# idiap/IdiapTTS

Hardware: AMD Instinct MI355X
Metric: acoustic frames/sec (train) (higher is better)
Workload: dtype f32

## Files before the change

idiaptts_amd/csrc/nn.hip:

```cpp
#include <algorithm>
#include <cstdlib>

#include "common.h"
#include "gemm_ring.h"
#include "gemm_staged.h"

namespace itts {

constexpr int BN = 128;

template <bool ROWFORM, bool VEC, int NROWS>
__device__ __forceinline__ void load_tile(const float* __restrict__ P, int64_t ld, int64_t out0,
                                          int64_t out_dim, int64_t k0, int64_t k_end,
                                          float4 (&r)[NROWS / 32]) {
  const int tid = threadIdx.x;
#pragma unroll
  for (int i = 0; i < NROWS / 32; ++i) {
    const int idx = tid + 256 * i;
    int64_t o, k;
    if (ROWFORM) {
      o = out0 + (idx >> 3);
      k = k0 + ((idx & 7) << 2);
    } else {
      k = k0 + idx / (NROWS / 4);
      o = out0 + ((idx % (NROWS / 4)) << 2);
    }
    const int64_t c = ROWFORM ? k : o, c_end = ROWFORM ? k_end : out_dim;
    const int64_t t = ROWFORM ? o : k, t_end = ROWFORM ? out_dim : k_end;
    const bool t_ok = t < t_end;
    const int64_t tc = t_ok ? t : 0;
    if (VEC) {
      const bool ok = t_ok && (c < c_end);
      const float4 v = *reinterpret_cast<const float4*>(P + tc * ld + (ok ? c : 0));
// ... 219 lines not shown
static int ring_wm(int64_t M, int N) {
  const double w2 = (double)(((M + 127) / 128) * 128) * (double)(((N + 63) / 64) * 64);
  const double w1 = (double)(((M + 63) / 64) * 64) * (double)(((N + 127) / 128) * 128);
  return w1 < w2 ? 1 : 2;
}

template <bool A_ROW, bool B_ROW, int EPI, int AF>
static int launch_ring(const GemmArgs& g, int splitk, hipStream_t s) {
  if (ring_wm(g.M, g.N) == 1) return launch_ring_wm<A_ROW, B_ROW, EPI, 1, AF>(g, splitk, s);
  return launch_ring_wm<A_ROW, B_ROW, EPI, 2, AF>(g, splitk, s);
}

template <int WM_W, int EPI_X, int AF_X = AF_BASE>
static int launch_ring_bwd_pair(const GemmArgs& gw, int splitk, const GemmArgs& gx, hipStream_t s) {
  const ring::Args rw = ring_args<WM_W>(gw, splitk), rx = ring_args<2>(gx, 1);
  hipLaunchKernelGGL((ring::gemm_ring_pair_kernel<false, false, EPI_STORE, WM_W, true, false, EPI_X, 2, AF_X>),
                     dim3(kRingGrid), dim3(ring::THREADS), 0, s, rw, rx);
  ITTS_LAUNCH_CHECK();
  return ITTS_OK;
}

template <bool A_ROW, bool B_ROW, int EPI, int AF = AF_BASE>
static int launch_gemm(GemmArgs g, int splitk, hipStream_t s) {
  if (g.M <= 0 || g.N <= 0) return ITTS_OK;
  if (ring_ok<A_ROW, B_ROW>(g, splitk, EPI)) return launch_ring<A_ROW, B_ROW, EPI, AF>(g, splitk, s);
  if (A_ROW) return launch_gemm_tn<A_ROW, B_ROW, EPI, 1, 1, AF>(g, splitk, s);
  const double e2 = tile_efficiency(g.M, g.N, splitk, 2, 1.0);
  const double e1 = tile_efficiency(g.M, g.N, splitk, 1, 0.90);
  if (e1 > e2) return launch_gemm_tn<A_ROW, B_ROW, EPI, 1, 2, AF>(g, splitk, s);
  return launch_gemm_tn<A_ROW, B_ROW, EPI, 2, 2, AF>(g, splitk, s);
}


__device__ __forceinline__ void reduce_slabs_vec_body(const float* __restrict__ slabs, int S, int64_t n,
                                                      float* __restrict__ out, int accumulate, int64_t block,
                                                      float4 (*part)[64]) {
  const int tx = threadIdx.x & 63, grp = threadIdx.x >> 6;
  const int64_t n4 = n >> 2;
  const int64_t c = block * 64 + tx;
  float4 s = make_float4(0.f, 0.f, 0.f, 0.f);
  if (c < n4) {
    const float4* p = reinterpret_cast<const float4*>(slabs) + c;
#pragma unroll 8
    for (int z = grp; z < S; z += 4) {
      const float4 v = p[(int64_t)z * n4];
      s.x += v.x; s.y += v.y; s.z += v.z; s.w += v.w;
    }
  }
  if (grp > 0) part[grp - 1][tx] = s;
  __syncthreads();
  if (grp == 0 && c < n4) {
#pragma unroll
    for (int g2 = 0; g2 < 3; ++g2) {
      const float4 v = part[g2][tx];
      s.x += v.x; s.y += v.y; s.z += v.z; s.w += v.w;
    }
    float4* o = reinterpret_cast<float4*>(out) + c;
    if (accumulate) {
      const float4 v = *o;
      s.x += v.x; s.y += v.y; s.z += v.z; s.w += v.w;
    }
    *o = s;
  }
}

__device__ __forceinline__ void reduce_slabs_scalar_body(const float* __restrict__ slabs, int S, int64_t n,
                                                         float* __restrict__ out, int accumulate,
                                                         int64_t block, float (*part)[64]) {
  const int tx = threadIdx.x & 63, grp = threadIdx.x >> 6;
  const int64_t c = block * 64 + tx;
  float s = 0.f;
  if (c < n) {
#pragma unroll 8
    for (int z = grp; z < S; z += 4) s += slabs[(int64_t)z * n + c];
  }
  if (grp > 0) part[grp - 1][tx] = s;
  __syncthreads();
  if (grp == 0 && c < n) {
    s += part[0][tx];
    s += part[1][tx];
    s += part[2][tx];
    out[c] = accumulate ? out[c] + s : s;
  }
}

__global__ __launch_bounds__(256) void reduce_slabs_kernel(const float* __restrict__ slabs, int S,
                                                           int64_t n, float* __restrict__ out,
                                                           int accumulate) {
  __shared__ float4 part[3][64];
  reduce_slabs_vec_body(slabs, S, n, out, accumulate, blockIdx.x, part);
}

__global__ __launch_bounds__(256) void reduce_slabs_scalar_kernel(const float* __restrict__ slabs, int S,
                                                                  int64_t n, float* __restrict__ out,
                                                                  int accumulate) {
  __shared__ float part[3][64];
  reduce_slabs_scalar_body(slabs, S, n, out, accumulate, blockIdx.x, part);
}

constexpr int kMaxDeferred = 16;
struct ReduceSeg {
  const void* src;
  void* out;
  int64_t n;
  double scale;
  int S;
  int accumulate;
  int kind;
  int first_block;
};
struct ReduceMulti {
  ReduceSeg seg[kMaxDeferred];
  int nseg;
};

__global__ __launch_bounds__(256) void reduce_multi_kernel(ReduceMulti d) {
  __shared__ float4 part4[3][64];
  __shared__ double red[16];
  int i = 0;
  while (i + 1 < d.nseg && (int)blockIdx.x >= d.seg[i + 1].first_block) ++i;
  const ReduceSeg& g = d.seg[i];
  const int64_t block = (int64_t)blockIdx.x - g.first_block;
  if (g.kind == 0) {
    reduce_slabs_vec_body(static_cast<const float*>(g.src), g.S, g.n, static_cast<float*>(g.out), g.accumulate,
                          block, part4);
  } else if (g.kind == 1) {
    reduce_slabs_scalar_body(static_cast<const float*>(g.src), g.S, g.n, static_cast<float*>(g.out),
                             g.accumulate, block, reinterpret_cast<float (*)[64]>(part4));
  } else {
    const double* partial = static_cast<const double*>(g.src);
    double s = 0.0;
    for (int k = threadIdx.x; k < (int)g.n; k += 256) s += partial[k];
    s = block_sum(s, red);
    if (threadIdx.x == 0) *static_cast<float*>(g.out) = (float)(s * g.scale);
  }
}

static thread_local bool t_defer = false;
static thread_local ReduceMulti t_pending{};

static int flush_deferred(hipStream_t s) {
  if (t_pending.nseg == 0) return ITTS_OK;
  const ReduceSeg& last = t_pending.seg[t_pending.nseg - 1];
  const int64_t per = last.kind == 0 ? (last.n / 4 + 63) / 64 : (last.kind == 1 ? (last.n + 63) / 64 : 1);
  const int64_t blocks = last.first_block + per;
  hipLaunchKernelGGL(reduce_multi_kernel, dim3((unsigned)blocks), dim3(256), 0, s, t_pending);
  t_pending.nseg = 0;
  ITTS_LAUNCH_CHECK();
  return ITTS_OK;
}

static int queue_deferred(ReduceSeg g, hipStream_t s) {
  if (t_pending.nseg == kMaxDeferred) {
    const int rc = flush_deferred(s);
    if (rc) return rc;
  }
  int64_t first = 0;
  if (t_pending.nseg > 0) {
    const ReduceSeg& p = t_pending.seg[t_pending.nseg - 1];
    first = p.first_block + (p.kind == 0 ? (p.n / 4 + 63) / 64 : (p.kind == 1 ? (p.n + 63) / 64 : 1));
  }
  ITTS_REQUIRE(first < ((int64_t)1 << 30), "too many deferred reduction blocks");
  g.first_block = (int)first;
  t_pending.seg[t_pending.nseg++] = g;
  return ITTS_OK;
}

static int launch_reduce_slabs(const float* slabs, int S, int64_t n, float* out, int accumulate,
                               hipStream_t s) {
  const bool vec = n % 4 == 0 && aligned16(slabs) && aligned16(out);
  if (t_defer) {
    ReduceSeg g{};
    g.src = slabs; g.out = out; g.n = n; g.S = S; g.accumulate = accumulate; g.kind = vec ? 0 : 1;
    return queue_deferred(g, s);
  }
  if (vec)
    hipLaunchKernelGGL(reduce_slabs_kernel, dim3((unsigned)((n / 4 + 63) / 64)), dim3(256), 0, s, slabs, S,
                       n, out, accumulate);
  else
    hipLaunchKernelGGL(reduce_slabs_scalar_kernel, dim3((unsigned)((n + 63) / 64)), dim3(256), 0, s, slabs,
                       S, n, out, accumulate);
  ITTS_LAUNCH_CHECK();
  return ITTS_OK;
}

extern "C" int itts_defer_reductions(int on) {
  ITTS_REQUIRE(on || t_pending.nseg == 0,
               "queued reductions must be run (itts_reduce_deferred) before deferral is switched off");
  t_defer = on != 0;
  return ITTS_OK;
}

extern "C" int itts_reduce_deferred(void* stream) {
  t_defer = false;
  return flush_deferred(as_stream(stream));
}

template <int AF>
__global__ void act_bwd_kernel(const float* __restrict__ dy, const float* __restrict__ y,
                               float* __restrict__ dz, int64_t n, int act) {
  if (AF == AF_BASE) {
    for (int64_t i = blockIdx.x * (int64_t)blockDim.x + threadIdx.x; i < n;
         i += (int64_t)gridDim.x * blockDim.x)
      dz[i] = dy[i] * act_grad_from_out(y[i], act);
  } else {
    with_ext_act(act, [&](auto a) {
      for (int64_t i = blockIdx.x * (int64_t)blockDim.x + threadIdx.x; i < n;
           i += (int64_t)gridDim.x * blockDim.x)
        dz[i] = dy[i] * dact1<decltype(a)::value>(y[i]);
    });
  }
}

__global__ __launch_bounds__(256) void masked_mse_kernel(
    const float* __restrict__ pred, int64_t ldp, const float* __restrict__ target, int64_t ldt,
    const uint8_t* __restrict__ valid, int64_t M, int D, float gscale, float* __restrict__ grad,
    int64_t ldg, double* __restrict__ partial) {
  __shared__ double red[16];
  const int64_t n = M * D;
  double s = 0.0;
  for (int64_t i = blockIdx.x * (int64_t)blockDim.x + threadIdx.x; i < n;
       i += (int64_t)gridDim.x * blockDim.x) {
    const int64_t r = i / D;
    const int c = (int)(i - r * D);
    float diff = 0.f;
    if (valid[r]) diff = pred[r * ldp + c] - target[r * ldt + c];
    s += (double)diff * (double)diff;
    if (grad) grad[r * ldg + c] = gscale * diff;
// ... 16 lines not shown
  if (t_defer) {
    ReduceSeg g{};
    g.src = partial; g.out = loss; g.n = nb; g.scale = scale; g.S = 1; g.kind = 2;
    return queue_deferred(g, s);
  }
  hipLaunchKernelGGL(masked_mse_final_kernel, dim3(1), dim3(256), 0, s, partial, nb, scale, loss);
  ITTS_LAUNCH_CHECK();
  return ITTS_OK;
}


__global__ __launch_bounds__(256) void weighted_loss_kernel(
    const float* __restrict__ pred, int64_t ldp, const float* __restrict__ target, int64_t ldt,
    const float* __restrict__ w, int64_t M, int D, int kind, float* __restrict__ grad, int64_t ldg,
    float* __restrict__ elem, int64_t lde, double* __restrict__ partial) {
  __shared__ double red[16];
  const int64_t n = M * D;
  double s = 0.0;
  for (int64_t i = blockIdx.x * (int64_t)blockDim.x + threadIdx.x; i < n;
       i += (int64_t)gridDim.x * blockDim.x) {
    const int64_t r = i / D;
    const int c = (int)(i - r * D);
    const float wr = w[r];
    const float diff = pred[r * ldp + c] - target[r * ldt + c];
    const float e = kind == 0 ? diff * diff : fabsf(diff);
    const float g = kind == 0 ? 2.f * diff : (diff > 0.f ? 1.f : (diff < 0.f ? -1.f : 0.f));
    const float v = wr == 0.f ? 0.f : wr * e;
    s += (double)v;
    if (grad) grad[r * ldg + c] = wr == 0.f ? 0.f : wr * g;
    if (elem) elem[r * lde + c] = v;
  }
  s = block_sum(s, red);
  if (threadIdx.x == 0) partial[blockIdx.x] = s;
}

__global__ void adam_kernel(float* __restrict__ p, const float* __restrict__ g,
                            float* __restrict__ m, float* __restrict__ v, int64_t n, float beta1,
                            float beta2, float eps, float wd, float step_size, float bc2_sqrt,
                            float gscale) {
  for (int64_t i = blockIdx.x * (int64_t)blockDim.x + threadIdx.x; i < n;
       i += (int64_t)gridDim.x * blockDim.x) {
    float gi = g[i] * gscale;
    float pi = p[i];
    if (wd != 0.f) gi += wd * pi;
    float mi = m[i], vi = v[i];
    mi = mi + (gi - mi) * (1.f - beta1);
    vi = vi * beta2 + (1.f - beta2) * gi * gi;
    const float denom = sqrtf(vi) / bc2_sqrt + eps;
    pi = pi - step_size * (mi / denom);
    p[i] = pi;
    m[i] = mi;
    v[i] = vi;
  }
}

__global__ void adam_fused_kernel(float* __restrict__ p, const float* __restrict__ g,
                                  float* __restrict__ m, float* __restrict__ v, int64_t n,
                                  float beta1, float beta2, float eps, float wd, float step_size,
                                  float bc2_sqrt, float gscale, const float* __restrict__ norm_accum,
                                  int norm_kind, float max_norm, float clip_value,
                                  float* __restrict__ shadow, float one_minus_decay) {
  float coef = gscale;
  if (norm_accum) {
    const float a = norm_accum[0];
    const float total = (norm_kind == 2 ? sqrtf(a) : a) * fabsf(gscale);
    coef *= fminf(1.f, max_norm / (total + 1e-6f));
  }
  for (int64_t i = blockIdx.x * (int64_t)blockDim.x + threadIdx.x; i < n;
       i += (int64_t)gridDim.x * blockDim.x) {
    float gi = g[i] * coef;
    if (clip_value > 0.f) gi = fminf(fmaxf(gi, -clip_value), clip_value);
    float pi = p[i];
    if (wd != 0.f) gi += wd * pi;
    float mi = m[i], vi = v[i];
    mi = mi + (gi - mi) * (1.f - beta1);
    vi = vi * beta2 + (1.f - beta2) * gi * gi;
    const float denom = sqrtf(vi) / bc2_sqrt + eps;
    pi = pi - step_size * (mi / denom);
    p[i] = pi;
    m[i] = mi;
    v[i] = vi;
    if (shadow) {
      const float si = shadow[i];
      shadow[i] = si - one_minus_decay * (si - pi);
    }
  }
// ... 360 lines not shown
  return launch_mse_final(reinterpret_cast<const double*>(d_workspace), nb, scale, d_loss, s);
}

extern "C" int itts_weighted_loss(const float* d_pred, int64_t ldp, const float* d_target, int64_t ldt,
                                  const float* d_row_weight, int64_t M, int D, int kind,
                                  float* d_loss, float* d_grad, int64_t ldg, float* d_elem,
                                  int64_t lde, void* d_workspace, void* stream) {
  ITTS_REQUIRE(d_pred && d_target && d_row_weight && d_loss && d_workspace, "null pointer");
  ITTS_REQUIRE(M >= 0 && D > 0 && ldp >= D && ldt >= D && (kind == 0 || kind == 1), "bad sizes");
  ITTS_REQUIRE((!d_grad || ldg >= D) && (!d_elem || lde >= D), "leading dimension too small");
  hipStream_t s = as_stream(stream);
  if (M == 0) {
    ITTS_HIP_CHECK(hipMemsetAsync(d_loss, 0, 4, s));
    return ITTS_OK;
  }
  const int nb = mse_blocks(M, D);
  hipLaunchKernelGGL(weighted_loss_kernel, dim3(nb), dim3(256), 0, s, d_pred, ldp, d_target, ldt,
                     d_row_weight, M, D, kind, d_grad, ldg, d_elem, lde,
                     reinterpret_cast<double*>(d_workspace));
  ITTS_LAUNCH_CHECK();
  hipLaunchKernelGGL(masked_mse_final_kernel, dim3(1), dim3(256), 0, s,
                     reinterpret_cast<const double*>(d_workspace), nb, 1.0, d_loss);
  ITTS_LAUNCH_CHECK();
  return ITTS_OK;
}

extern "C" int itts_adam_step(float* d_param, const float* d_grad, float* d_exp_avg,
                              float* d_exp_avg_sq, int64_t n, float lr, float beta1, float beta2,
                              float eps, float weight_decay, int64_t step, float grad_scale,
                              void* stream) {
  ITTS_REQUIRE(d_param && d_grad && d_exp_avg && d_exp_avg_sq, "null pointer");
  ITTS_REQUIRE(n >= 0 && step >= 1, "bad sizes (step counts from 1)");
  if (n == 0) return ITTS_OK;
  const double bc1 = 1.0 - pow((double)beta1, (double)step);
  const double bc2 = 1.0 - pow((double)beta2, (double)step);
  const float step_size = (float)((double)lr / bc1);
  const float bc2_sqrt = (float)sqrt(bc2);
  const int blocks = (int)std::min<int64_t>((n + 255) / 256, 4096);
  hipLaunchKernelGGL(adam_kernel, dim3(blocks), dim3(256), 0, as_stream(stream), d_param, d_grad,
                     d_exp_avg, d_exp_avg_sq, n, beta1, beta2, eps, weight_decay, step_size,
                     bc2_sqrt, grad_scale);
  ITTS_LAUNCH_CHECK();
  return ITTS_OK;
}

extern "C" int itts_grad_norm_accum(const float* d_x, int64_t n, int norm_kind, float* d_accum,
                                    int accumulate, void* d_workspace, void* stream) {
  ITTS_REQUIRE(d_accum && d_workspace && (n == 0 || d_x), "null pointer");
  ITTS_REQUIRE(n >= 0 && (norm_kind == 2 || norm_kind == 0), "norm_kind must be 2 or 0 (infinity)");
  const int nb = (int)std::min<int64_t>((n + 255) / 256, kNormBlocks);
  hipStream_t s = as_stream(stream);
  float* part = static_cast<float*>(d_workspace);
  if (nb > 0) {
    hipLaunchKernelGGL(grad_norm_partial_kernel, dim3(nb), dim3(256), 0, s, d_x, n, norm_kind, part);
    ITTS_LAUNCH_CHECK();
  }
  hipLaunchKernelGGL(grad_norm_final_kernel, dim3(1), dim3(256), 0, s, part, nb, norm_kind, d_accum,
                     accumulate);
  ITTS_LAUNCH_CHECK();
  return ITTS_OK;
}

extern "C" int itts_adam_step_fused(float* d_param, const float* d_grad, float* d_exp_avg,
                                    float* d_exp_avg_sq, int64_t n, float lr, float beta1,
                                    float beta2, float eps, float weight_decay, int64_t step,
                                    float grad_scale, const float* d_norm_accum, int norm_kind,
                                    float clip_max_norm, float clip_value, float* d_ema_shadow,
                                    float ema_decay, void* stream) {
  ITTS_REQUIRE(d_param && d_grad && d_exp_avg && d_exp_avg_sq, "null pointer");
  ITTS_REQUIRE(n >= 0 && step >= 1, "bad sizes (step counts from 1)");
  ITTS_REQUIRE(!d_norm_accum || ((norm_kind == 2 || norm_kind == 0) && clip_max_norm > 0.f),
               "norm clipping needs norm_kind 2 or 0 and a positive max norm");
  if (n == 0) return ITTS_OK;
  const double bc1 = 1.0 - pow((double)beta1, (double)step);
  const double bc2 = 1.0 - pow((double)beta2, (double)step);
  const int blocks = (int)std::min<int64_t>((n + 255) / 256, 4096);
// ... 35 lines not shown
```

idiaptts_amd/lib.py:

```python
import ctypes
import os
from ctypes import POINTER, c_char_p, c_double, c_float, c_int, c_int64, c_uint8, c_void_p

_HERE = os.path.dirname(os.path.abspath(__file__))
LIB_PATH = os.path.join(_HERE, "_lib", "libidiaptts_amd.so")

_lib = None


class IttsError(RuntimeError):
    pass


_P = c_void_p

_SIGNATURES = {
    "itts_abi_version": (c_int, []),
    "itts_last_error": (c_char_p, []),
    "itts_device_count": (c_int, []),
    "itts_release_scratch": (c_int, []),
    "itts_defer_reductions": (c_int, [c_int]),
    "itts_reduce_deferred": (c_int, [_P]),
    "itts_scratch_pool_stats": (c_int, [POINTER(c_int64), POINTER(c_int64), POINTER(c_int64)]),
    "itts_comm_version": (c_int, []),
    "itts_comm_unique_id": (c_int, [_P]),
    "itts_comm_init_rank": (c_int, [_P, c_int, c_int, POINTER(c_void_p)]),
    "itts_comm_destroy": (c_int, [c_void_p]),
    "itts_allreduce_flat": (c_int, [_P, c_int64, c_int, c_int, c_void_p, _P]),
    "itts_cheaptrick_fft_size": (c_int, [c_int, c_double]),
    "itts_num_aperiodicities": (c_int, [c_int]),
    "itts_mcep_alpha": (c_double, [c_int]),
    "itts_world_num_frames": (c_int64, [c_int64, c_int, c_double]),
    "itts_world_synth_length": (c_int64, [c_int64, c_int, c_double]),
    "itts_wav_info": (c_int, [c_char_p, POINTER(c_int), POINTER(c_int64)]),
    "itts_wav_read_batch": (c_int, [POINTER(c_char_p), c_int, POINTER(c_int64), c_double, _P,
                                    c_int]),
    "itts_write_feature_archives": (c_int, [_P, c_int64, POINTER(c_int64), c_int,
                                            POINTER(c_char_p), c_int, POINTER(c_int),
                                            POINTER(c_int), POINTER(c_int), POINTER(c_char_p),
                                            c_int, _P]),
    "itts_questions_load": (c_int, [c_char_p, POINTER(c_void_p), POINTER(c_int), POINTER(c_int)]),
    "itts_questions_free": (None, [c_void_p]),
    "itts_questions_vector": (c_int, [c_void_p, c_char_p, _P]),
    "itts_labels_count_frames": (c_int, [POINTER(c_char_p), c_int, POINTER(c_int64), c_int]),
    "itts_labels_generate": (c_int, [c_void_p, POINTER(c_char_p), c_int, POINTER(c_int64), _P,
                                     c_int64, c_int]),
    "itts_normalise_rows_f32": (c_int, [_P, c_int64, c_int, _P, _P, _P]),
    "itts_mlpg_scratch_bytes": (c_int64, [c_int64, c_int]),
    "itts_mlpg_generation": (c_int, [_P, c_int64, c_int, c_int, _P, POINTER(c_int64), c_int, _P,
                                     c_int64, c_int, _P, _P]),
    "itts_mlpg_scratch_bytes_f32": (c_int64, [c_int64, c_int]),
    "itts_mlpg_generation_f32": (c_int, [_P, c_int64, c_int, c_int, _P, POINTER(c_int64), c_int, _P,
                                         c_int64, c_int, _P, _P]),
    "itts_lf0_vuv": (c_int, [_P, POINTER(c_int64), c_int, c_double, c_float, _P, _P, _P]),
    "itts_interpolate_lin_f32": (c_int, [_P, POINTER(c_int64), c_int, _P, _P, _P]),
# ... 184 lines not shown
```

idiaptts_amd/native_ff.py:

```python
import math

import torch

from . import ops


def _pad4(n):
    return (n + 3) // 4 * 4


class FlatFFModel:

    def __init__(self, dims=(425, 512, 512, 187), acts=("tanh", "tanh", None), device="cuda",
                 seed=0, state_dict=None):
        assert len(acts) == len(dims) - 1
        self.dims = tuple(int(d) for d in dims)
        self.acts = [ops.act_code(a) for a in acts]
        self.device = torch.device(device)
        self.in_pitch = _pad4(self.dims[0])
        self.layout = []
        off = 0
        for li, (K, N) in enumerate(zip(self.dims[:-1], self.dims[1:])):
            kp = _pad4(K) if li == 0 else K
            w_off = off
# ... 71 lines not shown

    def bias(self, i, buf=None):
        _, b_off, N, _, _ = self.layout[i]
        return (self.params if buf is None else buf)[b_off:b_off + N]

    def pack_input(self, x):
        if x.shape[1] == self.in_pitch:
            return x
        xp = torch.zeros((x.shape[0], self.in_pitch), dtype=torch.float32, device=x.device)
        xp[:, :x.shape[1]] = x
        return xp

    def layers(self):
        return [(self.weight(i).clone(), self.bias(i).clone()) for i in range(len(self.layout))]

    def _rows_buffer(self, name, M, width):
        pitch = _pad4(width)
        buf = self._buffers.get(name)
        if buf is None or buf.shape[0] < M:
            buf = torch.zeros((M, pitch), dtype=torch.float32, device=self.device)
            self._buffers[name] = buf
        return buf[:M, :width]

    def forward(self, x, n_layers=None):
        acts = []
        h = self.pack_input(x)
        M = h.shape[0]
        for i in range(len(self.layout) if n_layers is None else n_layers):
            h = ops.linear_fwd(h, self.weight_padded(i), self.bias(i), self.acts[i],
                               out=self._rows_buffer("h%d" % i, M, self.layout[i][2]))
            acts.append(h)
        return acts

    def loss_and_backward(self, x, target, row_valid, n_valid_global, reduce_group=None, reduce=False):
        self._pending = []
        x = self.pack_input(x)
        if reduce:
            return self._loss_and_backward(x, target, row_valid, n_valid_global, reduce_group, reduce)
        with ops.deferred_reductions():
            return self._loss_and_backward(x, target, row_valid, n_valid_global, reduce_group, False)

    def _loss_and_backward(self, x, target, row_valid, n_valid_global, reduce_group, reduce):
        M = x.shape[0]
        n = len(self.layout)
        if self.acts[-1] in (None, ops.ACT_NONE) and n > 1:
            hs = self.forward(x, n_layers=n - 1)
            loss, dz = ops.linear_fwd_mse(hs[-1], self.weight_padded(n - 1), self.bias(n - 1), target,
                                          row_valid, n_valid_global,
                                          grad=self._rows_buffer("dz_out", M, self.dims[-1]))
            hs.append(None)
        else:
            hs = self.forward(x)
            loss, dz = ops.masked_mse(hs[-1], target, row_valid, n_valid_global,
                                      grad=self._rows_buffer("dz_out", M, self.dims[-1]))
            if self.acts[-1] != ops.ACT_NONE:
                dz = ops.act_bwd(dz, hs[-1], self.acts[-1])
        for i in range(n - 1, -1, -1):
            inp = hs[i - 1] if i > 0 else x
            dz_in = None
            if i > 0:
                dz_in = self._rows_buffer("dz%d" % (i & 1), M, self.layout[i][3])
                ops.linear_bwd(dz, inp, self.weight_padded(i), self.weight_padded(i, self.grads),
                               self.bias(i, self.grads), dz_in, yprev=hs[i - 1], act_prev=self.acts[i - 1])
            else:
                ops.linear_bwd_weight(dz, inp, dw=self.weight_padded(i, self.grads),
                                      db=self.bias(i, self.grads))
            if reduce:
                from .parallel import allreduce_flat_
                w_off, b_off, N, _, _ = self.layout[i]
                work = allreduce_flat_(self.grads[w_off:b_off + _pad4(N)], reduce_group, async_op=True)
                if work is not None:
                    self._pending.append(work)
            if i > 0:
                dz = dz_in
        return loss

    def train_step(self, x, target, row_valid, n_valid_global, lr=1e-3, betas=(0.9, 0.999),
                   eps=1e-8, weight_decay=0.0, process_group=None, world_size=1,
                   clip_norm_kind=None, clip_max_norm=0.0, clip_value=None, ema_shadow=None,
                   ema_decay=0.0):
        from . import parallel
        dist_on = world_size > 1 or parallel._active(process_group)
        loss = self.loss_and_backward(x, target, row_valid, n_valid_global, reduce_group=process_group,
                                      reduce=dist_on)
        for work in self._pending:
            work.wait()
        self._pending = []
        self.step_count += 1
        if clip_norm_kind is None and not clip_value and ema_shadow is None:
            ops.adam_step(self.params, self.grads, self.exp_avg, self.exp_avg_sq, self.step_count,
                          lr=lr, betas=betas, eps=eps, weight_decay=weight_decay)
            return loss
        accum = None
        if clip_norm_kind is not None:
            if getattr(self, "_norm_accum", None) is None:
                self._norm_accum = torch.zeros(1, dtype=torch.float32, device=self.device)
            accum = ops.grad_norm_accum(self.grads, self._norm_accum, clip_norm_kind)
        ops.adam_step_fused(self.params, self.grads, self.exp_avg, self.exp_avg_sq,
                            self.step_count, lr=lr, betas=betas, eps=eps,
                            weight_decay=weight_decay, norm_accum=accum,
                            norm_kind=clip_norm_kind if clip_norm_kind is not None else 2,
                            clip_max_norm=clip_max_norm, clip_value=clip_value or 0.0,
                            ema_shadow=ema_shadow, ema_decay=ema_decay)
        return loss


def flops_per_frame(dims, skip_first_dgrad=True):
    f = 0
    for i, (K, N) in enumerate(zip(dims[:-1], dims[1:])):
        f += 2 * N * K * (2 if (i == 0 and skip_first_dgrad) else 3)
    return f
```

idiaptts_amd/ops.py:

```python
import collections
import contextlib
import ctypes
import threading

import torch

from . import lib as _lib

ACT_NONE, ACT_TANH, ACT_RELU = 0, 1, 2
(ACT_SIGMOID, ACT_LOGSIGMOID, ACT_SOFTPLUS, ACT_SOFTSIGN, ACT_LEAKY_RELU, ACT_ELU, ACT_CELU, ACT_SELU, ACT_HARDTANH,
 ACT_RELU6, ACT_HARDSIGMOID) = range(3, 14)
ACT_TORCH_NAME = {ACT_TANH: "Tanh", ACT_RELU: "ReLU", ACT_SIGMOID: "Sigmoid", ACT_LOGSIGMOID: "LogSigmoid",
                  ACT_SOFTPLUS: "Softplus", ACT_SOFTSIGN: "Softsign", ACT_LEAKY_RELU: "LeakyReLU", ACT_ELU: "ELU",
                  ACT_CELU: "CELU", ACT_SELU: "SELU", ACT_HARDTANH: "Hardtanh", ACT_RELU6: "ReLU6",
                  ACT_HARDSIGMOID: "Hardsigmoid"}
ACT_BY_NAME = {None: ACT_NONE, "none": ACT_NONE, "linear": ACT_NONE}
ACT_BY_NAME.update({name.lower(): code for code, name in ACT_TORCH_NAME.items()})
CONV_ACTS = (ACT_NONE, ACT_TANH, ACT_RELU)


def act_code(act, allowed=None, where="Linear"):
    code = act if isinstance(act, int) else ACT_BY_NAME.get(act.lower() if isinstance(act, str) else act)
    if code is None or code not in (allowed if allowed is not None else range(ACT_HARDSIGMOID + 1)):
        raise NotImplementedError("{} activation {!r} is not implemented".format(where, act))
# ... 474 lines not shown
    if out is None:
        out = torch.empty((M, K), dtype=torch.float32, device=dz.device)
    _lib.check(L.itts_linear_bwd_input(_ptr(dz), _rows(dz, "dz"), _ptr(w), _ptr(out),
                                       _rows(out, "out"), _ptr(yprev),
                                       _rows(yprev, "yprev") if yprev is not None else 0,
                                       act_prev, M, N, K, _stream()), "itts_linear_bwd_input")
    return out


_ws_cache = {}
class _DeferState(threading.local):
    on = False
    next = 0


_defer = _DeferState()


def _workspace(nbytes, device):
    key = (device.index if device.index is not None else torch.cuda.current_device(),
           torch.cuda.current_stream(device).cuda_stream)
    if _defer.on:
        key = key + (_defer.next,)
        _defer.next += 1
    buf = _ws_cache.get(key)
    if buf is None or buf.numel() < nbytes:
        buf = torch.empty(max(int(nbytes), 1 << 20), dtype=torch.uint8, device=device)
        _ws_cache[key] = buf
    return buf


class deferred_reductions:

    def __enter__(self):
        if _defer.on:
            raise RuntimeError("deferred_reductions() blocks do not nest")
        _lib.check(_lib.load().itts_defer_reductions(1), "itts_defer_reductions")
        _defer.on, _defer.next = True, 0
        return self

    def __exit__(self, exc_type, exc, tb):
        _defer.on = False
        _lib.check(_lib.load().itts_reduce_deferred(_stream()), "itts_reduce_deferred")
        return False


def linear_bwd_weight(dz, x, dw=None, db=None, accumulate=False, want_bias=True):
    L = _lib.load()
    _need(dz, torch.float32, "dz")
    _need(x, torch.float32, "x")
    M, N = dz.shape
    K = x.shape[1]
    if dw is None:
        dw = torch.empty((N, K), dtype=torch.float32, device=dz.device)
    if db is None and want_bias:
        db = torch.empty((N,), dtype=torch.float32, device=dz.device)
    ws = _workspace(L.itts_linear_bwd_weight_workspace_bytes(M, N, K), dz.device)
    _lib.check(L.itts_linear_bwd_weight(_ptr(dz), _rows(dz, "dz"), _ptr(x), _rows(x, "x"),
                                        _ptr(dw), _ptr(db), M, N, K, _ptr(ws),
                                        1 if accumulate else 0, _stream()),
               "itts_linear_bwd_weight")
    return dw, db


def conv1d_out_len(T_in, kernel_size, padding, dilation):
    return T_in + 2 * padding - dilation * (kernel_size - 1)


def _conv_rows(t, name):
    if t.dim() != 3:
        raise ValueError("{} must be 3-D [B, T, C] (batch_first) or [T, B, C]".format(name))
    C = t.shape[2]
    ld = t.stride(1) if t.shape[1] > 1 else (t.stride(0) if t.shape[0] > 1 else C)
    ok = (t.stride(2) == 1 or C == 1) and ld >= C and (t.shape[0] == 1 or t.stride(0) == t.shape[1] * ld)
    if ok and ld != C and ld % 4 == 0:
        ok = t.storage_offset() + t.shape[0] * t.shape[1] * ld <= t.untyped_storage().nbytes() // 4
# ... 196 lines not shown


def grad_norm_accum(x, accum, norm_kind=2, accumulate=False):
    L = _lib.load()
    _need(x, torch.float32, "x")
    _need(accum, torch.float32, "accum")
    if not x.is_contiguous():
        raise ValueError("x must be contiguous")
    _lib.check(L.itts_grad_norm_accum(_ptr(x), x.numel(), int(norm_kind), _ptr(accum),
                                      int(bool(accumulate)), _ptr(_workspace(4096, x.device)),
                                      _stream()), "itts_grad_norm_accum")
    return accum


def adam_step_fused(param, grad, exp_avg, exp_avg_sq, step, lr=1e-3, betas=(0.9, 0.999), eps=1e-8,
                    weight_decay=0.0, grad_scale=1.0, norm_accum=None, norm_kind=2,
                    clip_max_norm=0.0, clip_value=0.0, ema_shadow=None, ema_decay=0.0):
    L = _lib.load()
    for t, n in ((param, "param"), (grad, "grad"), (exp_avg, "exp_avg"),
                 (exp_avg_sq, "exp_avg_sq")) + \
            (((ema_shadow, "ema_shadow"),) if ema_shadow is not None else ()):
        _need(t, torch.float32, n)
        if not t.is_contiguous() or t.numel() != param.numel():
            raise ValueError(n + " must be contiguous and as long as param")
    _lib.check(L.itts_adam_step_fused(
        _ptr(param), _ptr(grad), _ptr(exp_avg), _ptr(exp_avg_sq), param.numel(), lr, betas[0],
        betas[1], eps, weight_decay, int(step), grad_scale,
        _ptr(norm_accum) if norm_accum is not None else None, int(norm_kind),
        float(clip_max_norm), float(clip_value or 0.0),
        _ptr(ema_shadow) if ema_shadow is not None else None, float(ema_decay), _stream()),
        "itts_adam_step_fused")


def sgd_step(param, grad, momentum_buf=None, first_step=False, lr=1e-3, momentum=0.0,
             dampening=0.0, weight_decay=0.0, nesterov=False, grad_scale=1.0):
    L = _lib.load()
    for t, n in ((param, "param"), (grad, "grad")) + \
            (((momentum_buf, "momentum_buf"),) if momentum_buf is not None else ()):
        _need(t, torch.float32, n)
        if not t.is_contiguous():
            raise ValueError(n + " must be contiguous")
    _lib.check(L.itts_sgd_step(_ptr(param), _ptr(grad),
                               _ptr(momentum_buf) if momentum_buf is not None else None,
                               param.numel(), lr, momentum, dampening, weight_decay,
                               int(bool(nesterov)), int(bool(first_step)), grad_scale,
                               _stream()), "itts_sgd_step")


def ema_update(shadow, param, decay):
    L = _lib.load()
    for t, n in ((shadow, "shadow"), (param, "param")):
        _need(t, torch.float32, n)
        if not t.is_contiguous():
            raise ValueError(n + " must be contiguous")
    _lib.check(L.itts_ema_update(_ptr(shadow), _ptr(param), shadow.numel(), float(decay),
                                 _stream()), "itts_ema_update")


RnnPathCounts = collections.namedtuple("RnnPathCounts", "fwd_ran fwd_declined fwd_gave_up bwd_ran bwd_declined bwd_gave_up")


def rnn_path_counts():
    out = (ctypes.c_int64 * 6)()
    _lib.check(_lib.load().itts_rnn_path_counts(out), "itts_rnn_path_counts")
    return RnnPathCounts(*[int(v) for v in out])

# ... 250 lines not shown
```

include/idiaptts_amd.h:

```cpp
#ifndef IDIAPTTS_AMD_H
#define IDIAPTTS_AMD_H

#include <stdint.h>

#ifdef __cplusplus
extern "C" {
#endif

#define ITTS_OK 0
#define ITTS_E_INVALID (-1)
#define ITTS_E_HIP (-2)
#define ITTS_E_UNSUPPORTED (-3)

int itts_abi_version(void);
const char* itts_last_error(void);
int itts_device_count(void);
int itts_scratch_pool_stats(int64_t* reserved, int64_t* used, int64_t* keep_threshold);

int itts_release_scratch(void);

int itts_defer_reductions(int on);
int itts_reduce_deferred(void* stream);

#define ITTS_F32 0
#define ITTS_F64 1
#define ITTS_REDUCE_SUM 0
#define ITTS_REDUCE_MAX 1
#define ITTS_REDUCE_AVG 2
int itts_comm_version(void);
int itts_comm_unique_id(void* h_id128);
int itts_comm_init_rank(const void* h_id128, int n_ranks, int rank, void** comm_out);
int itts_comm_destroy(void* comm);
int itts_allreduce_flat(void* d_buf, int64_t n, int dtype, int op, void* comm, void* stream);

int itts_cheaptrick_fft_size(int fs, double f0_floor);
int itts_num_aperiodicities(int fs);
double itts_mcep_alpha(int fs);
int64_t itts_world_num_frames(int64_t n_samples, int fs, double frame_period_ms);
int64_t itts_world_synth_length(int64_t n_frames, int fs, double frame_period_ms);

int itts_wav_info(const char* h_path, int* fs, int64_t* n_samples);
int itts_wav_read_batch(const char* const* h_paths, int n_files, const int64_t* h_offsets,
                        double preemphasis, double* h_out, int n_threads);
int itts_write_feature_archives(const float* h_feat, int64_t ld, const int64_t* h_f_off, int n_utts,
                                const char* const* h_paths, int n_streams, const int* h_col0,
                                const int* h_width, const int* h_parts, const char* const* h_keys,
                                int n_threads, unsigned char* h_needs_merge);

int itts_normalise_rows_f32(const float* h_x, int64_t rows, int cols, const double* h_sub,
                            const double* h_div, float* h_out);

int itts_questions_load(const char* h_path, void** handle, int* n_binary, int* n_continuous);
void itts_questions_free(void* handle);
int itts_questions_vector(void* handle, const char* h_label, double* h_out);
int itts_labels_count_frames(const char* const* h_paths, int n_files, int64_t* h_frames, int n_threads);
// ... 260 lines not shown
```

Baseline: 37.84 million.

## Fuse deferred gradient slab reductions with the Adam update into one launch

```diff
diff --git a/idiaptts_amd/csrc/nn.hip b/idiaptts_amd/csrc/nn.hip
--- a/idiaptts_amd/csrc/nn.hip
+++ b/idiaptts_amd/csrc/nn.hip
@@ -1,4 +1,5 @@
 #include <algorithm>
+#include <atomic>
 #include <cstdlib>
 
 #include "common.h"
@@ -284,13 +285,39 @@
 }
 
 
-__device__ __forceinline__ void reduce_slabs_vec_body(const float* __restrict__ slabs, int S, int64_t n,
-                                                      float* __restrict__ out, int accumulate, int64_t block,
-                                                      float4 (*part)[64]) {
+struct AdamCoef {
+  float beta1, beta2, eps, wd, step_size, bc2_sqrt;
+};
+__device__ __forceinline__ void adam_update(float& pi, float& mi, float& vi, float gi, const AdamCoef& a) {
+  if (a.wd != 0.f) gi += a.wd * pi;
+  mi = mi + (gi - mi) * (1.f - a.beta1);
+  vi = vi * a.beta2 + (1.f - a.beta2) * gi * gi;
+  const float denom = sqrtf(vi) / a.bc2_sqrt + a.eps;
+  pi = pi - a.step_size * (mi / denom);
+}
+
+__global__ void adam_kernel(float* __restrict__ p, const float* __restrict__ g,
+                            float* __restrict__ m, float* __restrict__ v, int64_t n, float beta1,
+                            float beta2, float eps, float wd, float step_size, float bc2_sqrt,
+                            float gscale) {
+  const AdamCoef a{beta1, beta2, eps, wd, step_size, bc2_sqrt};
+  for (int64_t i = blockIdx.x * (int64_t)blockDim.x + threadIdx.x; i < n;
+       i += (int64_t)gridDim.x * blockDim.x) {
+    float pi = p[i], mi = m[i], vi = v[i];
+    adam_update(pi, mi, vi, g[i] * gscale, a);
+    p[i] = pi;
+    m[i] = mi;
+    v[i] = vi;
+  }
+}
+
+__device__ __forceinline__ bool reduce_slabs_vec_sum(const float* __restrict__ slabs, int S, int64_t n,
+                                                     const float* __restrict__ out, int accumulate, int64_t block,
+                                                     float4 (*part)[64], float4& s, int64_t& c) {
   const int tx = threadIdx.x & 63, grp = threadIdx.x >> 6;
   const int64_t n4 = n >> 2;
-  const int64_t c = block * 64 + tx;
-  float4 s = make_float4(0.f, 0.f, 0.f, 0.f);
+  c = block * 64 + tx;
+  s = make_float4(0.f, 0.f, 0.f, 0.f);
   if (c < n4) {
     const float4* p = reinterpret_cast<const float4*>(slabs) + c;
 #pragma unroll 8
@@ -301,39 +328,53 @@
   }
   if (grp > 0) part[grp - 1][tx] = s;
   __syncthreads();
-  if (grp == 0 && c < n4) {
+  if (grp != 0 || c >= n4) return false;
 #pragma unroll
-    for (int g2 = 0; g2 < 3; ++g2) {
-      const float4 v = part[g2][tx];
-      s.x += v.x; s.y += v.y; s.z += v.z; s.w += v.w;
-    }
-    float4* o = reinterpret_cast<float4*>(out) + c;
-    if (accumulate) {
-      const float4 v = *o;
-      s.x += v.x; s.y += v.y; s.z += v.z; s.w += v.w;
-    }
-    *o = s;
-  }
+  for (int g2 = 0; g2 < 3; ++g2) {
+    const float4 v = part[g2][tx];
+    s.x += v.x; s.y += v.y; s.z += v.z; s.w += v.w;
+  }
+  if (accumulate) {
+    const float4 v = reinterpret_cast<const float4*>(out)[c];
+    s.x += v.x; s.y += v.y; s.z += v.z; s.w += v.w;
+  }
+  return true;
+}
+
+__device__ __forceinline__ void reduce_slabs_vec_body(const float* __restrict__ slabs, int S, int64_t n,
+                                                      float* __restrict__ out, int accumulate, int64_t block,
+                                                      float4 (*part)[64]) {
+  float4 s;
+  int64_t c;
+  if (reduce_slabs_vec_sum(slabs, S, n, out, accumulate, block, part, s, c)) reinterpret_cast<float4*>(out)[c] = s;
+}
+
+__device__ __forceinline__ bool reduce_slabs_scalar_sum(const float* __restrict__ slabs, int S, int64_t n,
+                                                        const float* __restrict__ out, int accumulate,
+                                                        int64_t block, float (*part)[64], float& s, int64_t& c) {
+  const int tx = threadIdx.x & 63, grp = threadIdx.x >> 6;
+  c = block * 64 + tx;
+  s = 0.f;
+  if (c < n) {
+#pragma unroll 8
+    for (int z = grp; z < S; z += 4) s += slabs[(int64_t)z * n + c];
+  }
+  if (grp > 0) part[grp - 1][tx] = s;
+  __syncthreads();
+  if (grp != 0 || c >= n) return false;
+  s += part[0][tx];
+  s += part[1][tx];
+  s += part[2][tx];
+  s = accumulate ? out[c] + s : s;
+  return true;
 }
 
 __device__ __forceinline__ void reduce_slabs_scalar_body(const float* __restrict__ slabs, int S, int64_t n,
                                                          float* __restrict__ out, int accumulate,
                                                          int64_t block, float (*part)[64]) {
-  const int tx = threadIdx.x & 63, grp = threadIdx.x >> 6;
-  const int64_t c = block * 64 + tx;
-  float s = 0.f;
-  if (c < n) {
-#pragma unroll 8
-    for (int z = grp; z < S; z += 4) s += slabs[(int64_t)z * n + c];
-  }
-  if (grp > 0) part[grp - 1][tx] = s;
-  __syncthreads();
-  if (grp == 0 && c < n) {
-    s += part[0][tx];
-    s += part[1][tx];
-    s += part[2][tx];
-    out[c] = accumulate ? out[c] + s : s;
-  }
+  float s;
+  int64_t c;
+  if (reduce_slabs_scalar_sum(slabs, S, n, out, accumulate, block, part, s, c)) out[c] = s;
 }
 
 __global__ __launch_bounds__(256) void reduce_slabs_kernel(const float* __restrict__ slabs, int S,
@@ -361,10 +402,21 @@
   int kind;
   int first_block;
 };
+static int64_t seg_blocks(const ReduceSeg& g) {
+  return g.kind == 0 ? (g.n / 4 + 63) / 64 : g.kind == 1 ? (g.n + 63) / 64 : g.kind == 2 ? 1 : (g.n + 255) / 256;
+}
 struct ReduceMulti {
   ReduceSeg seg[kMaxDeferred];
   int nseg;
 };
+
+__device__ __forceinline__ void reduce_partials_body(const ReduceSeg& g, double* red) {
+  const double* partial = static_cast<const double*>(g.src);
+  double s = 0.0;
+  for (int k = threadIdx.x; k < (int)g.n; k += 256) s += partial[k];
+  s = block_sum(s, red);
+  if (threadIdx.x == 0) *static_cast<float*>(g.out) = (float)(s * g.scale);
+}
 
 __global__ __launch_bounds__(256) void reduce_multi_kernel(ReduceMulti d) {
   __shared__ float4 part4[3][64];
@@ -380,11 +432,72 @@
     reduce_slabs_scalar_body(static_cast<const float*>(g.src), g.S, g.n, static_cast<float*>(g.out),
                              g.accumulate, block, reinterpret_cast<float (*)[64]>(part4));
   } else {
-    const double* partial = static_cast<const double*>(g.src);
-    double s = 0.0;
-    for (int k = threadIdx.x; k < (int)g.n; k += 256) s += partial[k];
-    s = block_sum(s, red);
-    if (threadIdx.x == 0) *static_cast<float*>(g.out) = (float)(s * g.scale);
+    reduce_partials_body(g, red);
+  }
+}
+
+struct AdamFlat {
+  float* p;
+  const float* g;
+  float* m;
+  float* v;
+  AdamCoef c;
+  int64_t adam_off[kMaxDeferred];
+};
+
+__global__ __launch_bounds__(256) void reduce_multi_adam_kernel(ReduceMulti d, AdamFlat a) {
+  __shared__ float4 part4[3][64];
+  __shared__ double red[16];
+  int i = 0;
+  while (i + 1 < d.nseg && (int)blockIdx.x >= d.seg[i + 1].first_block) ++i;
+  const ReduceSeg& g = d.seg[i];
+  const int64_t block = (int64_t)blockIdx.x - g.first_block;
+  const int64_t off = a.adam_off[i];
+  if (g.kind == 0) {
+    float4 s;
+    int64_t c;
+    if (reduce_slabs_vec_sum(static_cast<const float*>(g.src), g.S, g.n, static_cast<const float*>(g.out),
+                             g.accumulate, block, part4, s, c)) {
+      static_cast<float4*>(g.out)[c] = s;
+      if (off >= 0) {
+        float4* p4 = reinterpret_cast<float4*>(a.p + off) + c;
+        float4* m4 = reinterpret_cast<float4*>(a.m + off) + c;
+        float4* v4 = reinterpret_cast<float4*>(a.v + off) + c;
+        float4 pv = *p4, mv = *m4, vv = *v4;
+        adam_update(pv.x, mv.x, vv.x, s.x, a.c);
+        adam_update(pv.y, mv.y, vv.y, s.y, a.c);
+        adam_update(pv.z, mv.z, vv.z, s.z, a.c);
+        adam_update(pv.w, mv.w, vv.w, s.w, a.c);
+        *p4 = pv;
+        *m4 = mv;
+        *v4 = vv;
+      }
+    }
+  } else if (g.kind == 1) {
+    float s;
+    int64_t c;
+    if (reduce_slabs_scalar_sum(static_cast<const float*>(g.src), g.S, g.n, static_cast<const float*>(g.out),
+                                g.accumulate, block, reinterpret_cast<float (*)[64]>(part4), s, c)) {
+      static_cast<float*>(g.out)[c] = s;
+      if (off >= 0) {
+        float pi = a.p[off + c], mi = a.m[off + c], vi = a.v[off + c];
+        adam_update(pi, mi, vi, s, a.c);
+        a.p[off + c] = pi;
+        a.m[off + c] = mi;
+        a.v[off + c] = vi;
+      }
+    }
+  } else if (g.kind == 2) {
+    reduce_partials_body(g, red);
+  } else {
+    const int64_t c = block * 256 + threadIdx.x;
+    if (c < g.n) {
+      float pi = a.p[off + c], mi = a.m[off + c], vi = a.v[off + c];
+      adam_update(pi, mi, vi, a.g[off + c], a.c);
+      a.p[off + c] = pi;
+      a.m[off + c] = mi;
+      a.v[off + c] = vi;
+    }
   }
 }
 
@@ -394,8 +507,7 @@
 static int flush_deferred(hipStream_t s) {
   if (t_pending.nseg == 0) return ITTS_OK;
   const ReduceSeg& last = t_pending.seg[t_pending.nseg - 1];
-  const int64_t per = last.kind == 0 ? (last.n / 4 + 63) / 64 : (last.kind == 1 ? (last.n + 63) / 64 : 1);
-  const int64_t blocks = last.first_block + per;
+  const int64_t blocks = last.first_block + seg_blocks(last);
   hipLaunchKernelGGL(reduce_multi_kernel, dim3((unsigned)blocks), dim3(256), 0, s, t_pending);
   t_pending.nseg = 0;
   ITTS_LAUNCH_CHECK();
@@ -410,7 +522,7 @@
   int64_t first = 0;
   if (t_pending.nseg > 0) {
     const ReduceSeg& p = t_pending.seg[t_pending.nseg - 1];
-    first = p.first_block + (p.kind == 0 ? (p.n / 4 + 63) / 64 : (p.kind == 1 ? (p.n + 63) / 64 : 1));
+    first = p.first_block + seg_blocks(p);
   }
   ITTS_REQUIRE(first < ((int64_t)1 << 30), "too many deferred reduction blocks");
   g.first_block = (int)first;
@@ -446,6 +558,90 @@
 extern "C" int itts_reduce_deferred(void* stream) {
   t_defer = false;
   return flush_deferred(as_stream(stream));
+}
+
+static int launch_adam(float* p, const float* g, float* m, float* v, int64_t n, const AdamCoef& c, float gscale,
+                       hipStream_t s) {
+  const int blocks = (int)std::min<int64_t>((n + 255) / 256, 4096);
+  hipLaunchKernelGGL(adam_kernel, dim3(blocks), dim3(256), 0, s, p, g, m, v, n, c.beta1, c.beta2, c.eps, c.wd,
+                     c.step_size, c.bc2_sqrt, gscale);
+  ITTS_LAUNCH_CHECK();
+  return ITTS_OK;
+}
+
+static std::atomic<int64_t> g_tail_fused{0}, g_tail_two_launches{0};
+
+static AdamCoef adam_coef(float lr, float beta1, float beta2, float eps, float wd, int64_t step) {
+  const double bc1 = 1.0 - pow((double)beta1, (double)step);
+  const double bc2 = 1.0 - pow((double)beta2, (double)step);
+  return AdamCoef{beta1, beta2, eps, wd, (float)((double)lr / bc1), (float)sqrt(bc2)};
+}
+
+extern "C" int itts_reduce_deferred_adam(float* d_param, float* d_grad, float* d_exp_avg, float* d_exp_avg_sq,
+                                         int64_t n, int64_t step, float lr, float beta1, float beta2, float eps,
+                                         float weight_decay, void* stream) {
+  t_defer = false;
+  hipStream_t s = as_stream(stream);
+  const bool args_ok = d_param && d_grad && d_exp_avg && d_exp_avg_sq && n >= 0 && step >= 1;
+  if (!args_ok) flush_deferred(s);
+  ITTS_REQUIRE(d_param && d_grad && d_exp_avg && d_exp_avg_sq, "null pointer");
+  ITTS_REQUIRE(n >= 0 && step >= 1, "bad sizes (step counts from 1)");
+  if (n == 0) return flush_deferred(s);
+  const AdamCoef coef = adam_coef(lr, beta1, beta2, eps, weight_decay, step);
+  const char* sw = getenv("ITTS_FF_FUSED_TAIL");
+  bool fused = !(sw && sw[0] == '0') && aligned16(d_param) && aligned16(d_grad) && aligned16(d_exp_avg) &&
+               aligned16(d_exp_avg_sq);
+
+  ReduceMulti d = t_pending;
+  AdamFlat a{d_param, d_grad, d_exp_avg, d_exp_avg_sq, coef, {}};
+  struct Span { int64_t b, e; };
+  Span span[kMaxDeferred];
+  int nspan = 0;
+  for (int i = 0; i < d.nseg && fused; ++i) {
+    a.adam_off[i] = -1;
+    if (d.seg[i].kind == 2) continue;
+    const float* o = static_cast<const float*>(d.seg[i].out);
+    const float* oe = o + d.seg[i].n;
+    if (oe <= d_grad || o >= d_grad + n) continue;
+    if (o < d_grad || oe > d_grad + n) { fused = false; break; }
+    a.adam_off[i] = o - d_grad;
+    span[nspan++] = Span{o - d_grad, oe - d_grad};
+  }
+  std::sort(span, span + nspan, [](const Span& x, const Span& y) { return x.b < y.b; });
+  for (int i = 0; i + 1 < nspan; ++i) fused = fused && span[i].e <= span[i + 1].b;
+  int64_t at = 0;
+  for (int i = 0; i <= nspan && fused; ++i) {
+    const int64_t b = i < nspan ? span[i].b : n;
+    if (b > at) {
+      if (d.nseg == kMaxDeferred) { fused = false; break; }
+      const ReduceSeg& prev = d.seg[d.nseg > 0 ? d.nseg - 1 : 0];
+      const int64_t first = d.nseg > 0 ? prev.first_block + seg_blocks(prev) : 0;
+      ReduceSeg g{};
+      g.out = d_grad + at; g.n = b - at; g.kind = 3; g.first_block = (int)first;
+      a.adam_off[d.nseg] = at;
+      d.seg[d.nseg++] = g;
+    }
+    if (i < nspan) at = span[i].e;
+  }
+  const int64_t blocks = d.nseg > 0 ? d.seg[d.nseg - 1].first_block + seg_blocks(d.seg[d.nseg - 1]) : 0;
+  if (!fused || blocks >= ((int64_t)1 << 30)) {
+    g_tail_two_launches.fetch_add(1, std::memory_order_relaxed);
+    const int rc = flush_deferred(s);
+    if (rc) return rc;
+    return launch_adam(d_param, d_grad, d_exp_avg, d_exp_avg_sq, n, coef, 1.f, s);
+  }
+  t_pending.nseg = 0;
+  g_tail_fused.fetch_add(1, std::memory_order_relaxed);
+  hipLaunchKernelGGL(reduce_multi_adam_kernel, dim3((unsigned)blocks), dim3(256), 0, s, d, a);
+  ITTS_LAUNCH_CHECK();
+  return ITTS_OK;
+}
+
+extern "C" int itts_ff_tail_counts(int64_t out[2]) {
+  ITTS_REQUIRE(out, "null pointer");
+  out[0] = g_tail_fused.load(std::memory_order_relaxed);
+  out[1] = g_tail_two_launches.load(std::memory_order_relaxed);
+  return ITTS_OK;
 }
 
 template <int AF>
@@ -528,26 +724,6 @@
   }
   s = block_sum(s, red);
   if (threadIdx.x == 0) partial[blockIdx.x] = s;
-}
-
-__global__ void adam_kernel(float* __restrict__ p, const float* __restrict__ g,
-                            float* __restrict__ m, float* __restrict__ v, int64_t n, float beta1,
-                            float beta2, float eps, float wd, float step_size, float bc2_sqrt,
-                            float gscale) {
-  for (int64_t i = blockIdx.x * (int64_t)blockDim.x + threadIdx.x; i < n;
-       i += (int64_t)gridDim.x * blockDim.x) {
-    float gi = g[i] * gscale;
-    float pi = p[i];
-    if (wd != 0.f) gi += wd * pi;
-    float mi = m[i], vi = v[i];
-    mi = mi + (gi - mi) * (1.f - beta1);
-    vi = vi * beta2 + (1.f - beta2) * gi * gi;
-    const float denom = sqrtf(vi) / bc2_sqrt + eps;
-    pi = pi - step_size * (mi / denom);
-    p[i] = pi;
-    m[i] = mi;
-    v[i] = vi;
-  }
 }
 
 __global__ void adam_fused_kernel(float* __restrict__ p, const float* __restrict__ g,
@@ -974,16 +1150,8 @@
   ITTS_REQUIRE(d_param && d_grad && d_exp_avg && d_exp_avg_sq, "null pointer");
   ITTS_REQUIRE(n >= 0 && step >= 1, "bad sizes (step counts from 1)");
   if (n == 0) return ITTS_OK;
-  const double bc1 = 1.0 - pow((double)beta1, (double)step);
-  const double bc2 = 1.0 - pow((double)beta2, (double)step);
-  const float step_size = (float)((double)lr / bc1);
-  const float bc2_sqrt = (float)sqrt(bc2);
-  const int blocks = (int)std::min<int64_t>((n + 255) / 256, 4096);
-  hipLaunchKernelGGL(adam_kernel, dim3(blocks), dim3(256), 0, as_stream(stream), d_param, d_grad,
-                     d_exp_avg, d_exp_avg_sq, n, beta1, beta2, eps, weight_decay, step_size,
-                     bc2_sqrt, grad_scale);
-  ITTS_LAUNCH_CHECK();
-  return ITTS_OK;
+  return launch_adam(d_param, d_grad, d_exp_avg, d_exp_avg_sq, n, adam_coef(lr, beta1, beta2, eps, weight_decay, step),
+                     grad_scale, as_stream(stream));
 }
 
 extern "C" int itts_grad_norm_accum(const float* d_x, int64_t n, int norm_kind, float* d_accum,
diff --git a/idiaptts_amd/lib.py b/idiaptts_amd/lib.py
--- a/idiaptts_amd/lib.py
+++ b/idiaptts_amd/lib.py
@@ -21,6 +21,9 @@
     "itts_release_scratch": (c_int, []),
     "itts_defer_reductions": (c_int, [c_int]),
     "itts_reduce_deferred": (c_int, [_P]),
+    "itts_reduce_deferred_adam": (c_int, [_P, _P, _P, _P, c_int64, c_int64, c_float, c_float, c_float, c_float,
+                                          c_float, _P]),
+    "itts_ff_tail_counts": (c_int, [POINTER(c_int64)]),
     "itts_scratch_pool_stats": (c_int, [POINTER(c_int64), POINTER(c_int64), POINTER(c_int64)]),
     "itts_comm_version": (c_int, []),
     "itts_comm_unique_id": (c_int, [_P]),
diff --git a/idiaptts_amd/native_ff.py b/idiaptts_amd/native_ff.py
--- a/idiaptts_amd/native_ff.py
+++ b/idiaptts_amd/native_ff.py
@@ -127,12 +127,12 @@
             acts.append(h)
         return acts
 
-    def loss_and_backward(self, x, target, row_valid, n_valid_global, reduce_group=None, reduce=False):
+    def loss_and_backward(self, x, target, row_valid, n_valid_global, reduce_group=None, reduce=False, adam=None):
         self._pending = []
         x = self.pack_input(x)
         if reduce:
             return self._loss_and_backward(x, target, row_valid, n_valid_global, reduce_group, reduce)
-        with ops.deferred_reductions():
+        with ops.deferred_reductions(adam=adam):
             return self._loss_and_backward(x, target, row_valid, n_valid_global, reduce_group, False)
 
     def _loss_and_backward(self, x, target, row_valid, n_valid_global, reduce_group, reduce):
@@ -176,13 +176,20 @@
                    ema_decay=0.0):
         from . import parallel
         dist_on = world_size > 1 or parallel._active(process_group)
+        plain = clip_norm_kind is None and not clip_value and ema_shadow is None
+        adam = None
+        if plain and not dist_on:
+            adam = dict(param=self.params, grad=self.grads, exp_avg=self.exp_avg, exp_avg_sq=self.exp_avg_sq,
+                        step=self.step_count + 1, lr=lr, betas=betas, eps=eps, weight_decay=weight_decay)
         loss = self.loss_and_backward(x, target, row_valid, n_valid_global, reduce_group=process_group,
-                                      reduce=dist_on)
+                                      reduce=dist_on, adam=adam)
         for work in self._pending:
             work.wait()
         self._pending = []
         self.step_count += 1
-        if clip_norm_kind is None and not clip_value and ema_shadow is None:
+        if adam is not None:
+            return loss
+        if plain:
             ops.adam_step(self.params, self.grads, self.exp_avg, self.exp_avg_sq, self.step_count,
                           lr=lr, betas=betas, eps=eps, weight_decay=weight_decay)
             return loss
diff --git a/idiaptts_amd/ops.py b/idiaptts_amd/ops.py
--- a/idiaptts_amd/ops.py
+++ b/idiaptts_amd/ops.py
@@ -530,6 +530,15 @@
 
 class deferred_reductions:
 
+    def __init__(self, adam=None):
+        if adam is not None:
+            n = adam["param"].numel()
+            for k in ("param", "grad", "exp_avg", "exp_avg_sq"):
+                _need(adam[k], torch.float32, k)
+                if not adam[k].is_contiguous() or adam[k].numel() != n:
+                    raise ValueError(k + " must be contiguous and as long as param")
+        self.adam = adam
+
     def __enter__(self):
         if _defer.on:
             raise RuntimeError("deferred_reductions() blocks do not nest")
@@ -539,7 +548,15 @@
 
     def __exit__(self, exc_type, exc, tb):
         _defer.on = False
-        _lib.check(_lib.load().itts_reduce_deferred(_stream()), "itts_reduce_deferred")
+        a = self.adam
+        if a is None or exc_type is not None:
+            _lib.check(_lib.load().itts_reduce_deferred(_stream()), "itts_reduce_deferred")
+            return False
+        betas = a.get("betas", (0.9, 0.999))
+        _lib.check(_lib.load().itts_reduce_deferred_adam(
+            _ptr(a["param"]), _ptr(a["grad"]), _ptr(a["exp_avg"]), _ptr(a["exp_avg_sq"]), a["param"].numel(),
+            int(a["step"]), a.get("lr", 1e-3), betas[0], betas[1], a.get("eps", 1e-8), a.get("weight_decay", 0.0),
+            _stream()), "itts_reduce_deferred_adam")
         return False
 
 
@@ -802,6 +819,12 @@
         "itts_adam_step_fused")
 
 
+def ff_tail_counts():
+    out = (ctypes.c_int64 * 2)()
+    _lib.check(_lib.load().itts_ff_tail_counts(out), "itts_ff_tail_counts")
+    return int(out[0]), int(out[1])
+
+
 def sgd_step(param, grad, momentum_buf=None, first_step=False, lr=1e-3, momentum=0.0,
              dampening=0.0, weight_decay=0.0, nesterov=False, grad_scale=1.0):
     L = _lib.load()
diff --git a/include/idiaptts_amd.h b/include/idiaptts_amd.h
--- a/include/idiaptts_amd.h
+++ b/include/idiaptts_amd.h
@@ -21,6 +21,11 @@
 
 int itts_defer_reductions(int on);
 int itts_reduce_deferred(void* stream);
+
+int itts_reduce_deferred_adam(float* d_param, float* d_grad, float* d_exp_avg, float* d_exp_avg_sq,
+                              int64_t n, int64_t step, float lr, float beta1, float beta2, float eps,
+                              float weight_decay, void* stream);
+int itts_ff_tail_counts(int64_t out[2]);
 
 #define ITTS_F32 0
 #define ITTS_F64 1
```

Result: no change. 37.78 million (-0.2%).
